# turlando/flac-py

Hardware: AMD Instinct MI355X
Metric: PCM samples/sec encode-analysis, 4608-blk/16-bit mono, 1/2/4/8 MI355X (higher is better)
Workload: dtype i16 in; f64 autocorrelation/Levinson; i32 predictors; 1 GPU; 1e6 synthetic mono 4608-sample int16 blocks, -l 12 -q 5 -r 0,5; units_per_gpu=1000000, units_total=1000000, block=4608, sample_bits=16, max_lpc_order=12, qlp_precision=5, mode=reference, parallelism=dp1 (block shards), open_eighths=0, lpc_pruning=on: candidates proven to lose skipped (sign bound, partial-sum tiers)

## Files before the change

flac-py_amd/csrc/flacmi_host.cpp:

```cpp
#include <dlfcn.h>
#include <hip/hip_runtime.h>

#include <algorithm>
#include <atomic>
#include <cerrno>
#include <chrono>
#include <cmath>
#include <cstdarg>
#include <cstdio>
#include <cstdlib>
#include <cstring>
#include <map>
#include <mutex>
#include <string>
#include <vector>

#include "../../include/flacmi.h"
#include "flacmi_kernels.h"
#include "pymath.h"
#include "device_common.h"

using namespace flacmi;

static double (*volatile libm_cos)(double) = cos;
// ... 414 lines not shown
static int use_mfma() {
    static const int v = [] {
        const char* e = getenv("FLACMI_NO_MFMA");
        return (e && atoi(e) != 0) ? 0 : 1;
    }();
    return v;
}

static int use_stream() {
    static const int v = [] {
        const char* e = getenv("FLACMI_NO_STREAM");
        return (e && atoi(e) != 0) ? 0 : 1;
    }();
    return v;
}

static int sign_bound_allowed() {
    static const int v = [] {
        const char* e = getenv("FLACMI_NO_SIGNBOUND");
        return (e && atoi(e) != 0) ? 0 : 1;
    }();
    return v;
}

static int prune_allowed() {
    static const int v = [] {
        const char* e = getenv("FLACMI_NO_PRUNE");
        return (e && atoi(e) != 0) ? 0 : 1;
    }();
    return v;
}

constexpr int64_t kOverlapMinUnits = 16384;
static int overlap_mode() { return knob(kKnobOverlap); }

static int analyze_device_impl(flacmi_ctx* ctx, const flacmi_batch* b, const flacmi_params* p,
                               const flacmi_outputs* o, hipStream_t s, bool allow_overlap = true) {
    if (int rc = set_device(ctx)) return rc;
    const bool lpc = p->mode == FLACMI_MODE_REFERENCE || p->mode == FLACMI_MODE_LPC_ONLY;
    const int L = lpc ? p->max_lpc_order : 0;
    const int rec_words = FLACMI_LPC_REC_WORDS(L);
    if (lpc) {
        if (int rc = ensure_buf(ctx->rec, sizeof(int32_t) * (size_t)rec_words * (size_t)(b->n_units > 0 ? b->n_units : 1)))
            return rc;
    }
    const int energy = debug_stop() >= 11 ? 0 : knob(kKnobEnergyBound);
    const bool prune_call = p->mode == FLACMI_MODE_REFERENCE && !o->lpc_sums &&
                            !(p->reserved[1] & (FLACMI_FLAG_ALL_CANDIDATES | FLACMI_FLAG_LPC_SIGN)) && prune_allowed();
    const bool ebound = energy != 0 && prune_call && L >= 1 && L <= 12 && b->sample_bytes == 2 && p->qlp_precision <= 16;
    if (ebound) {
        if (int rc = ensure_buf(ctx->bound, sizeof(uint32_t) * 2 * (size_t)(b->n_units > 0 ? b->n_units : 1))) return rc;
    }
    constexpr int64_t kSubWords = 64 * 16;
    if (int rc = ensure_buf(ctx->retry, sizeof(int64_t) * (size_t)(kSubWords + 2 * b->n_units + 68))) return rc;
    struct Cls {
        int64_t unit0, count;
        int n;
    } cls[2];
    int ncls = 0;
    const int64_t nfull = b->n_units - b->n_tail_units;
    if (b->n_tail_units == 0 || b->tail_len == b->block_len) {
        cls[ncls++] = {0, b->n_units, b->block_len};
    } else {
        if (nfull > 0) cls[ncls++] = {0, nfull, b->block_len};
        cls[ncls++] = {nfull, b->n_tail_units, b->tail_len};
    }
// ... 26 lines not shown
                overlap = true;
                continue;
            }
        }
        int64_t k = overlap && ov > 1 ? cls[c].count / kOverlapMinUnits : 1;
        const int left = flacmi_ctx::kMaxChunks - nch - (ncls - 1 - c);
        k = k < 1 ? 1 : k > want ? want : k;
        k = k > left ? left : k;
        for (int64_t i = 0; i < k; ++i) {
            const int64_t u0 = cls[c].count * i / k, u1 = cls[c].count * (i + 1) / k;
            ch[nch++] = {cls[c].unit0 + u0, u1 - u0, cls[c].n};
        }
    }
    auto lpc_args = [&](const Chunk& k, LpcArgs& a) -> int {
        a = LpcArgs{};
        a.samples = b->samples;
        a.stride = b->unit_stride;
        a.unit0 = k.unit0;
        a.count = k.count;
        a.sample_bytes = b->sample_bytes;
        a.n = k.n;
        a.L = L;
        a.q = p->qlp_precision;
        a.lpc_sign = (p->reserved[1] & FLACMI_FLAG_LPC_SIGN) != 0;
        if (int rc = get_window(ctx, k.n, (double**)&a.window, &a.fuse_lo, &a.fuse_hi)) return rc;
        a.bound = ebound ? (uint32_t*)ctx->bound.p + 2 * k.unit0 : nullptr;
        if (b->sample_bits > 26) a.fuse_lo = a.fuse_hi = 0;
        a.log2thr = ctx->d_log2thr;
        a.rec = (int32_t*)ctx->rec.p + k.unit0 * rec_words;
        a.rec_words = rec_words;
        a.acf = o->acf ? o->acf + k.unit0 * 33 : nullptr;
        return 0;
    };
    auto launch_resid_chunk = [&](const Chunk& k, hipStream_t st) -> hipError_t {
        ResidArgs a{};
        a.samples = b->samples;
        a.stride = b->unit_stride;
        a.unit0 = k.unit0;
        a.count = k.count;
        a.sample_bytes = b->sample_bytes;
        a.n = k.n;
        a.L = L;
        a.mode = p->mode;
        a.rmin = p->rice_min;
        a.rmax = p->rice_max;
        a.rec = lpc ? (const int32_t*)ctx->rec.p + k.unit0 * rec_words : nullptr;
        a.rice_order = p->mode == FLACMI_MODE_RICE_ONLY ? p->reserved[0] : 0;
        a.rec_words = rec_words;
        a.log2thr = ctx->d_log2thr;
        a.meta = o->meta + k.unit0;
        a.rice_params = o->rice_params + k.unit0 * o->params_stride;
        a.params_stride = o->params_stride;
        a.residual = (char*)o->residual + (size_t)k.unit0 * o->residual_stride * o->residual_bytes;
        a.residual_stride = o->residual_stride;
        a.fixed_sums = o->fixed_sums ? o->fixed_sums + k.unit0 * 5 : nullptr;
        a.lpc_sums = o->lpc_sums ? o->lpc_sums + k.unit0 * 32 : nullptr;
        a.stop_after = debug_stop();
        a.mfma = use_mfma();
        int64_t* const rb = (int64_t*)ctx->retry.p;
        a.retry_sub = (unsigned long long*)rb;
        a.retry_count = (unsigned long long*)(rb + kSubWords);
        a.retry_list = rb + kSubWords + 2;
        a.retry2_count = (unsigned long long*)(rb + kSubWords + 2 + b->n_units + 64);
        a.retry2_list = rb + kSubWords + 4 + b->n_units + 64;
        a.sample_bits = b->sample_bits;
        a.stream = use_stream();
        a.prune = prune_call;
        if (ebound) {
            double* w = nullptr;
            if (get_window(ctx, k.n, &w, nullptr, nullptr, &a.chunk_weight)) return hipErrorOutOfMemory;
            a.bound = (const uint32_t*)ctx->bound.p + 2 * k.unit0;
            a.energy = energy;
        }
        a.sign_bound = !(p->reserved[1] & FLACMI_FLAG_TIERS_ONLY) && sign_bound_allowed();
        const bool wide = needs_wide(k.n, b->sample_bits, L, p->qlp_precision, p->mode);
        int path = (wide || o->residual_bytes == 8) ? 2 : (b->sample_bytes == 2 && p->qlp_precision <= 16) ? 0 : 1;
        if (path == 2 && o->residual_bytes == 4 && split_ok(b->sample_bits, L, p->qlp_precision)) path = 3;
        return launch_resid(a, path, o->residual_bytes, st);
    };
    const int slot = ctx->ncalls % flacmi_ctx::kRing;
    hipEvent_t* ev = ctx->ev[slot];
    hipStream_t side = nullptr;
    if (overlap && !allow_overlap) overlap = false;
    if (overlap) {
        if (int rc = enc_streams(ctx)) return rc;
        side = enc_side(ctx);
        if (side == s) overlap = false;
    }
    ctx->nchunks[slot] = overlap ? nch : 0;
    HIP_TRY(hipEventRecord(ev[0], s));
    if (overlap) {
        HIP_TRY(hipStreamWaitEvent(side, ev[0], 0));
        for (int i = 0; i < nch; ++i) {
            LpcArgs a;
            if (int rc = lpc_args(ch[i], a)) return rc;
            HIP_TRY(launch_lpc(a, side));
            HIP_TRY(hipEventRecord(ctx->lpc_done[i], side));
        }
        HIP_TRY(hipEventRecord(ev[1], side));
        for (int i = 0; i < nch; ++i) {
            HIP_TRY(hipStreamWaitEvent(s, ctx->lpc_done[i], 0));
            HIP_TRY(hipEventRecord(ev[3 + 2 * i], s));
            HIP_TRY(launch_resid_chunk(ch[i], s));
            HIP_TRY(hipEventRecord(ev[4 + 2 * i], s));
        }
    } else {
        for (int i = 0; i < nch && lpc; ++i) {
            LpcArgs a;
            if (int rc = lpc_args(ch[i], a)) return rc;
            HIP_TRY(launch_lpc(a, s));
        }
        HIP_TRY(hipEventRecord(ev[1], s));
        for (int i = 0; i < nch; ++i) HIP_TRY(launch_resid_chunk(ch[i], s));
    }
    HIP_TRY(hipEventRecord(ev[2], s));
    ctx->ncalls++;
    if (o->lpc_records) {
        if (lpc) {
            HIP_TRY(launch_expand_records((const int32_t*)ctx->rec.p, rec_words, L, b->n_units, o->lpc_records, s));
        } else {
            HIP_TRY(hipMemsetAsync(o->lpc_records, 0, sizeof(int32_t) * FLACMI_LPC_REC_WORDS(32) * b->n_units, s));
        }
    }
    return 0;
}

extern "C" {

int flacmi_analyze_device(flacmi_ctx* ctx, const flacmi_batch* batch, const flacmi_params* params,
                          const flacmi_outputs* out, void* stream) {
    if (!ctx) return fail(FLACMI_E_INVALID, "null context");
    if (int rc = validate(batch, params, out)) return rc;
    if (batch->n_units == 0) return 0;
    return analyze_device_impl(ctx, batch, params, out, (hipStream_t)stream);
}

int flacmi_analyze_host(flacmi_ctx* ctx, const flacmi_batch* batch, const flacmi_params* params,
// ... 1659 lines not shown
```

flac-py_amd/csrc/flacmi_kernels.h:

```cpp
#pragma once
#include <hip/hip_runtime.h>
#include <stdint.h>

#include "../../include/flacmi.h"

namespace flacmi {

constexpr int kWindowPad = 80;

struct LpcArgs {
    const void* samples;
    int64_t stride;
    int64_t unit0, count;
    int32_t sample_bytes;
    int32_t n, L, q;
    const double* window;
    const double* log2thr;
    int32_t* rec;
    int32_t rec_words;
    int32_t lpc_sign;
    double* acf;
    int32_t fuse_lo, fuse_hi;
    uint32_t* bound;
};
// ... 6 lines not shown
    const void* samples;
    int64_t stride;
    int64_t unit0, count;
    int32_t sample_bytes;
    int32_t n, L, mode;
    int32_t rmin, rmax;
    int32_t rice_order;
    const int32_t* rec;
    int32_t rec_words;
    const double* log2thr;
    flacmi_unit_meta* meta;
    int32_t* rice_params;
    int64_t params_stride;
    void* residual;
    int64_t residual_stride;
    int64_t* fixed_sums;
    int64_t* lpc_sums;
    int32_t stop_after;
    int32_t mfma;
    unsigned long long* retry_count;
    int64_t* retry_list;
    unsigned long long* retry2_count;
    int64_t* retry2_list;
    unsigned long long* retry_sub;
    int64_t retry_sub_cap;
    int32_t sample_bits;
    int32_t stream;
    int32_t prune;
    int32_t persist;
    int32_t sign_bound;
    const uint32_t* bound;
    const uint16_t* chunk_weight;
    int32_t energy;
};
#define FLACMI_STATUS_RETRY 0x7e

struct StereoChoice {
    int32_t code;
    int32_t status;
    int64_t unit[2];
};

struct FrameArgs {
    const void* samples;
    int64_t stride;
    int32_t sample_bytes;
    int32_t block_len, tail_len;
    int64_t n_units, n_tail_units;
    int32_t channels, sample_size, q;
    int64_t first_frame, n_frames;
    const flacmi_unit_meta* meta;
    const int32_t* rice_params;
    int64_t params_stride;
    const void* residual;
    int32_t residual_bytes;
    int64_t residual_stride;
    int64_t* offsets;
    int32_t* status;
    uint8_t* out;
    int64_t capacity;
    const uint16_t* crc_slice;
    const uint16_t* crc_pow;
    int32_t pack_split;
    unsigned long long* slow_count;
    int64_t* slow_list;
    int32_t ablate;
// ... 95 lines not shown
    uint8_t* parts;
    int32_t part_stride;
    const uint16_t* crc_slice;
    int32_t wasted_spec;
};

struct PcmArgs {
    const flacmi_pcm_frame* frames;
    int64_t n_frames;
    int32_t channels, bytes_per_sample, raw;
    uint8_t* out;
    int64_t capacity;
    int32_t* status;
};

struct ResidLaunch {
    int threads;
    size_t lds_bytes;
};

ResidLaunch resid_launch_config(int n, int rmax_eff, int residual_bytes);
constexpr int kMaxFinestParts = 4096;

enum Knob { kKnobOverlap = 0, kKnobMf8Grid, kKnobStreamGeneric, kKnobDecodeGeneric, kKnobPackGeneric, kKnobDecodeLpc, kKnobEnergyBound, kKnobInfoGrid, kKnobCount };
int knob(Knob k);

hipError_t launch_lpc(const LpcArgs& a, hipStream_t s);
int64_t lpc_units_per_round(const LpcArgs& a);
hipError_t launch_poison_lds(hipStream_t s);
hipError_t launch_export(const int64_t* off, const int32_t* st, int64_t nf, int64_t* h_off, int32_t* h_st,
                         hipStream_t s);
hipError_t launch_lpc_from_acf(const LpcArgs& a, hipStream_t s);
hipError_t launch_resid(const ResidArgs& a, int path, int residual_bytes, hipStream_t s);
hipError_t launch_expand_records(const int32_t* rec, int32_t rec_words, int32_t L, int64_t count,
                                 int32_t* out, hipStream_t s);
hipError_t launch_synth(void* dst, int32_t sample_bytes, int32_t bits, int64_t stride,
                        int64_t first_unit, int64_t n_units, int32_t len, uint64_t seed,
                        const int32_t* sintab, int32_t open8, hipStream_t s);
hipError_t launch_stats(const flacmi_unit_meta* meta, int64_t n_units, int32_t block_len,
                        int32_t tail_len, int64_t n_tail_units, int64_t* stats, hipStream_t s);

hipError_t launch_stereo_rows(const void* lr, int32_t sample_bytes, int64_t lr_stride, int64_t n_frames,
                              int32_t block_len, int32_t tail_len, int32_t has_tail, void* mid, int64_t mid_stride,
                              int32_t* side, int64_t side_stride, hipStream_t s);
hipError_t launch_wasted_rows(const void* in, int32_t sample_bytes, int64_t in_stride, int64_t n_units,
                              int32_t block_len, int32_t tail_len, int64_t n_tail_units, int32_t sample_bits,
                              void* out, int64_t out_stride, int32_t* wasted, hipStream_t s);
hipError_t launch_stereo_choose(const FrameArgs& a, hipStream_t s);

hipError_t launch_frame_sizes(const FrameArgs& a, int64_t* bsum, hipStream_t s);
int64_t frame_scan_blocks(int64_t n_frames);
hipError_t launch_pack(const FrameArgs& a, hipStream_t s);
hipError_t launch_decode(DecodeArgs a, hipStream_t s);
hipError_t launch_index(const IndexArgs& a, hipStream_t s);
hipError_t launch_frame_info(const InfoArgs& a, int grid_cap, hipStream_t s);
int64_t index_scan_groups(int64_t n_tiles);
hipError_t launch_pcm(const PcmArgs& a, hipStream_t s);

hipError_t launch_selftest(int32_t which, const double* x, double* out, int32_t* status, int64_t n,
                           const double* log2thr, hipStream_t s);

}
```

flac-py_amd/csrc/k_stream.hip:

```cpp
#include <type_traits>

#include "device_common.h"

namespace flacmi {

namespace {

typedef _Float16 h8 __attribute__((ext_vector_type(8)));
typedef float f4 __attribute__((ext_vector_type(4)));
typedef _Float16 h2 __attribute__((ext_vector_type(2)));
typedef unsigned short us2 __attribute__((ext_vector_type(2)));

#ifndef FLACMI_STREAM_CPT
#define FLACMI_STREAM_CPT 5
#endif
constexpr int kSCPT = FLACMI_STREAM_CPT;
#ifndef FLACMI_RICE_DEDUP
#define FLACMI_RICE_DEDUP 1
#endif
#ifndef FLACMI_SAD16
#define FLACMI_SAD16 1
#endif
__host__ __device__ constexpr int stream_threads(int n) {
    const int nch = n / 8;
    const int nt = 64 * ((nch + 64 * kSCPT - 1) / (64 * kSCPT));
    return nt < 64 ? 64 : nt;
}
constexpr int kSHP = 16;
constexpr uint32_t kMagicBits = 0x4B400000u;
constexpr int kRiceOrders = 8;

struct SLds {
    int xs, pk, rec, red, red2, red0, pks, total;
};

__host__ __device__ inline SLds stream_lds(int n, int nw, int tap_words, int P, int RS) {
    auto up = [](int b) { return (b + 15) & ~15; };
    auto mx = [](int x, int y) { return x > y ? x : y; };
    SLds l;
    int o = 0;
    l.xs = o;   o = up(o + 2 * (kSHP + n));
    l.pk = l.rec = o; o = up(o + mx(2 * P * RS, 4 * mx(tap_words, 1)));
    l.red = l.red2 = o; o = up(o + mx(8 * nw * 16, 8 * (nw + 1) * kRiceOrders));
    l.red0 = o; o = up(o + 8 * nw);
    l.pks = o;  o = up(o + 4 * P);
    l.total = o;
    return l;
}

__host__ __device__ constexpr int tap_table_words(int NG) { return NG > 0 ? 40 * NG + 1 : 0; }
__device__ __forceinline__ uint32_t f16_of_int(int v) {
    return (uint32_t)__builtin_bit_cast(unsigned short, (_Float16)(float)v);
}

constexpr uint32_t f16_bits(int v) {
    if (v == 0) return 0;
    const uint32_t sgn = v < 0 ? 0x8000u : 0u;
    const int m = v < 0 ? -v : v;
    int e = 0;
    while ((m >> (e + 1)) != 0) ++e;
    return sgn | (uint32_t)((e + 15) << 10) | (uint32_t)((m << (10 - e)) & 0x3ff);
}
constexpr int fixed_tap(int p, int j) {
    if (j == 0) return -1;
    if (j < 0 || j > p) return 0;
    int c = 1;
    for (int t = 0; t < j; ++t) c = c * (p - t) / (t + 1);
    return (j & 1) ? c : -c;
}
struct FixB {
    uint32_t w[64 * 4];
};
constexpr FixB make_fixb() {
    FixB t{};
    for (int l = 0; l < 64; ++l) {
        const int col = l & 15, kb = l >> 4, p = (col >> 2) + 1, rho = col & 3, ia = 12 + rho - 4 * kb;
        const int idx[2] = {ia, ia - 2};
        for (int k = 0; k < 2; ++k) {
            const int i = idx[k];
            t.w[4 * l + k] = f16_bits(256 * fixed_tap(p, i)) | f16_bits(256 * fixed_tap(p, i - 1)) << 16;
            t.w[4 * l + 2 + k] = f16_bits(fixed_tap(p, i)) | f16_bits(fixed_tap(p, i - 1)) << 16;
        }
    }
    return t;
}
__constant__ const FixB kFixB = make_fixb();

__device__ __forceinline__ uint32_t sad32(uint32_t a, uint32_t b, uint32_t acc) { return (a > b ? a - b : b - a) + acc; }
template <int CTRL>
__device__ __forceinline__ uint64_t dpp_min_u64(uint64_t v) {
    const uint32_t lo = (uint32_t)__builtin_amdgcn_update_dpp(0, (int)(uint32_t)v, CTRL, 0xf, 0xf, false);
    const uint32_t hi = (uint32_t)__builtin_amdgcn_update_dpp(0, (int)(uint32_t)(v >> 32), CTRL, 0xf, 0xf, false);
    const uint64_t o = ((uint64_t)hi << 32) | lo;
    return o < v ? o : v;
}
__device__ __forceinline__ uint32_t opaque(uint32_t v) {
    asm volatile("" : "+v"(v));
    return v;
}
__device__ __forceinline__ uint32_t opaque_s(uint32_t v) {
    asm volatile("" : "+s"(v));
    return v;
}

__device__ __forceinline__ uint32_t h2sub(uint32_t t, float c) {
    const h2 v = __builtin_bit_cast(h2, t) - h2{(_Float16)c, (_Float16)c};
    return __builtin_bit_cast(uint32_t, v);
}

__device__ __forceinline__ uint4 a_raw(uint2 q) {
    return uint4{__builtin_amdgcn_perm(0x64646464u, q.x, 0x04030401u), __builtin_amdgcn_perm(0x64646464u, q.y, 0x04030401u),
                 __builtin_amdgcn_perm(0x64646464u, q.x, 0x04020400u), __builtin_amdgcn_perm(0x64646464u, q.y, 0x04020400u)};
}
__device__ __forceinline__ h8 a_sub(uint4 r) {
    const uint4 v{h2sub(r.x, 1152.0f), h2sub(r.y, 1152.0f), h2sub(r.z, 1024.0f), h2sub(r.w, 1024.0f)};
    return __builtin_bit_cast(h8, v);
}

__device__ __forceinline__ int rice_param_exact(uint64_t s, int len) {
// ... 103 lines not shown

}

template <int NG, bool R05, int NFIX, bool LIST, bool EB, typename Args>
__device__ __forceinline__ void stream_unit(const Args& a, const int64_t gid, unsigned char* smem) {
    static_assert(!EB || (NG > 0 && !LIST), "the energy bound's build is the batch kernel's, in reference mode");
    const int tid = LIST ? (int)opaque((uint32_t)threadIdx.x) : (int)threadIdx.x, NT = NFIX ? stream_threads(NFIX) : (int)blockDim.x, lane = tid & 63, nw = NT >> 6;
#if FLACMI_STREAM_STAMPS
    uint64_t stamp[8];
    const uint64_t rt0 = __builtin_amdgcn_s_memrealtime();
    stamp[0] = __builtin_amdgcn_s_memtime();
#define STAMP(k) (stamp[k] = __builtin_amdgcn_s_memtime())
#else
#define STAMP(k) ((void)0)
#endif
    const int wid = __builtin_amdgcn_readfirstlane(tid >> 6);
    const int n = NFIX ? NFIX : a.n, L = NG > 0 ? (NFIX ? 4 * NG : a.L) : 0;
    const int nch = n >> 3, nblk = n >> 6;
    const int rw = NG > 0 ? (NFIX ? 2 + L + (L * (L + 1)) / 2 : a.rec_words) : 0;
    int rmax_eff = -1;
    for (int o = a.rmin; o <= a.rmax; ++o)
        if (n % (1 << o) == 0) rmax_eff = o;
    const int Pmax = 1 << rmax_eff;
    constexpr int RS = kRiceOrders;
    const SLds lay = stream_lds(n, nw, tap_table_words(NG), Pmax, RS);
    uint16_t* xs = reinterpret_cast<uint16_t*>(smem + lay.xs) + kSHP;
    int32_t* recl = reinterpret_cast<int32_t*>(smem + lay.rec);
    uint32_t* red0 = reinterpret_cast<uint32_t*>(smem + lay.red0);
    unsigned long long* red2 = reinterpret_cast<unsigned long long*>(smem + lay.red2);
    uint32_t* pks = reinterpret_cast<uint32_t*>(smem + lay.pks);
    uint16_t* pkw = reinterpret_cast<uint16_t*>(smem + lay.pk);
    flacmi_unit_meta* meta = a.meta + gid;
    MetaVals mv{};

    constexpr int kTW = tap_table_words(NG), kTJ = NG > 0 ? (kTW + 63) / 64 : 0;
    uint4 fixb;
    {
        const uint4* src = reinterpret_cast<const uint4*>((const int16_t*)a.samples + (a.unit0 + gid) * a.stride);
        uint4 q[kSCPT];
#pragma unroll
        for (int j = 0; j < kSCPT; ++j) {
#if FLACMI_NT_LOAD
            typedef unsigned int v4u __attribute__((ext_vector_type(4)));
            const v4u t = __builtin_nontemporal_load(reinterpret_cast<const v4u*>(src) + min(tid + j * NT, nch - 1));
            q[j] = uint4{t.x, t.y, t.z, t.w};
#else
            q[j] = src[min(tid + j * NT, nch - 1)];
#endif
        }
        fixb = reinterpret_cast<const uint4*>(kFixB.w)[lane];
        uint32_t cwv[EB ? kSCPT : 1];
        if constexpr (EB) {
#pragma unroll
            for (int j = 0; j < kSCPT; ++j) cwv[j] = a.chunk_weight[min(tid + j * NT, nch - 1)];
        }
        int32_t tv[kTJ > 0 ? kTJ : 1][2];
        if constexpr (NG > 0 && !EB) {
            const int32_t* r = a.rec + gid * rw;
#pragma unroll
            for (int j = 0; j < kTJ; ++j) {
                if (j > 0 && j * NT >= kTW) break;
                const int gw = tid + j * NT, p = gw / 10 + 1, w = gw - 10 * (p - 1);
                const int pc = p < L ? p : L, base = 2 + L + (pc * (pc - 1)) / 2;
                tv[j][0] = r[w == 8 ? 1 + pc : min(max(base + 15 - 2 * w, 0), rw - 1)];
                tv[j][1] = r[min(max(base + 14 - 2 * w, 0), rw - 1)];
            }
        }
        if (tid < kSHP) xs[tid - kSHP] = 0x8000u;
        if (tid < Pmax) pks[tid] = a.stop_after == 10 ? (uint32_t)n * 40u : 0u;
#if FLACMI_SAD16
        const uint32_t k8000 = opaque(0x80008000u);
#else
        const uint32_t k8000 = opaque(0x8000u);
#endif
        uint32_t sumx = 0, wsum = 0;
#pragma unroll
        for (int j = 0; j < kSCPT; ++j) {
            const int v = tid + j * NT;
            if (v < nch) {
                const uint4 y{q[j].x ^ 0x80008000u, q[j].y ^ 0x80008000u, q[j].z ^ 0x80008000u, q[j].w ^ 0x80008000u};
                *reinterpret_cast<uint4*>(xs + 8 * v) = y;
                const uint32_t yd[4] = {y.x, y.y, y.z, y.w};
                if constexpr (EB) {
// ... 14 lines not shown
#endif
                    }
                }
            }
        }
        if constexpr (NG > 0 && !EB) {
            uint32_t* tt = reinterpret_cast<uint32_t*>(recl);
#pragma unroll
            for (int j = 0; j < kTJ; ++j) {
                if (j > 0 && j * NT >= kTW) break;
                const int gw = tid + j * NT, p = gw / 10 + 1, w = gw - 10 * (p - 1);
                if (gw < kTW) {
                    auto tap = [&](int i, int32_t c) -> uint32_t {
                        if (p > L || i < 0 || i > p) return 0u;
                        return f16_of_int(i == 0 ? -(1 << c) : c);
                    };
                    tt[gw] = tap(16 - 2 * w, tv[j][0]) | tap(15 - 2 * w, tv[j][1]) << 16;
                }
            }
        }
        const uint32_t sx = wave_sum_u32(sumx);
        if (lane == 0) red0[wid] = sx;
        if constexpr (EB) {
            const uint32_t sw = wave_sum_u32(wsum >> 3);
            if (lane == 0) red0[nw + wid] = sw;
        }
    }
    STAMP(1);
    __syncthreads();
    STAMP(2);
    uint32_t negmask = 0;
    const int32_t* __restrict__ grec = NG > 0 ? a.rec + gid * rw : nullptr;
    if constexpr (NG > 0) {
        const int st = grec[0];
        if (st != 0) {
            if (wid == 0) {
                mv.status = st & 0xffff;
                mv.site = st >> 16;
                store_meta(meta, lane, mv, 0);
            }
            return;
        }
        if constexpr (!EB) negmask = (uint32_t)grec[1];
    }
    uint2 bw{0u, 0u};
    if constexpr (EB) bw = *reinterpret_cast<const uint2*>(a.bound + 2 * gid);
    const bool listed = EB && bw.x == kBoundUnusable && bw.y == kBoundOutside;

    const bool prune = EB || (NG > 0 && a.prune && !LIST);
    unsigned long long* red64 = reinterpret_cast<unsigned long long*>(smem + lay.red);
    auto lane_total = [&](bool with_lpc = true) __attribute__((always_inline)) -> uint64_t {
        uint64_t t = 0;
        int g = -1, o4l = 0;
        if (lane >= 1 && lane <= 4) {
            g = 0;
            o4l = lane - 1;
        } else if (NG > 0 && with_lpc && lane >= 16 && lane < 16 + 4 * NG) {
            g = 1 + ((lane - 16) >> 2);
            o4l = (lane - 16) & 3;
        }
        if (g >= 0) {
#pragma unroll 1
            for (int w2 = 0; w2 < nw; ++w2) t += red64[(w2 * 4 + g) * 4 + o4l];
        } else if (lane == 0) {
#pragma unroll 1
            for (int w2 = 0; w2 < nw; ++w2) t += red0[w2];
        }
        return t;
    };
    uint64_t tj = 0;
    bool pruned = false;
    {
        const int col = lane & 15, kb = lane >> 4, o4 = col >> 2, rho = col & 3;
        h8 B[NG + 1];
        int shg[NG + 1];
        const uint32_t* tt = reinterpret_cast<const uint32_t*>(recl);
        const int k0 = 4 + 4 * kb - rho;
        const uint32_t alb = 16u * (uint32_t)(k0 & 1);
        bool outside = false;
// ... 92 lines not shown
                            (g == 0 || !EX) ? sad32(bits, mbv, 0u) : lpc_abs(bits, shg[g], kgv, xn[r], 0u);
                        acc[g] += i >= start_of(g) ? sv : 0u;
                    } else if (g == 0 || !EX) {
                        acc[g] = opaque(sad32(bits, mbv, acc[g]));
                    } else {
                        acc[g] = lpc_abs(bits, shg[g], kgv, xn[r], acc[g]);
                    }
                }
            }
        };
        auto block = [&](auto g0c, auto g1c, auto exc, uint2 q, bool masked, int blk) __attribute__((always_inline)) {
            uint32_t xn[4];
            ldx(blk, xn);
            blockA(g0c, g1c, exc, a_raw(q), masked, xn);
        };
        const uint32_t xnone[4] = {0u, 0u, 0u, 0u};
        auto reduce_store = [&](auto g0c, auto bdc, auto g1c) __attribute__((always_inline)) {
            constexpr int G0 = decltype(g0c)::value, G1 = decltype(g1c)::value;
            constexpr bool BD = decltype(bdc)::value != 0;
#pragma unroll
            for (int g = G0; g <= G1; ++g) {
                uint32_t v = (BD && g > 0) ? acc[g] >> shg[g] : acc[g];
                v += (uint32_t)__builtin_amdgcn_update_dpp(0, (int)v, 0xB1, 0xf, 0xf, false);
                v += (uint32_t)__builtin_amdgcn_update_dpp(0, (int)v, 0x4E, 0xf, 0xf, false);
                uint64_t w = v;
                w += (uint64_t)(uint32_t)__builtin_amdgcn_ds_swizzle((int)v, 0x401F);
                w += __shfl_xor((unsigned long long)w, 32);
                if (rho == 0 && kb == 0) red64[(wid * 4 + g) * 4 + o4] = w;
            }
        };
        using I0 = std::integral_constant<int, 0>;
        using I1 = std::integral_constant<int, 1>;
        using ING = std::integral_constant<int, NG>;
        const int kw = (nblk - wid + nw - 1) / nw;
        if (EB && prune) {
            if (!listed) {
                for (int k = wid == 0 ? 1 : 0; k < kw; ++k) blockA(I0{}, I0{}, I0{}, a_raw(ld(wid + k * nw)), false, xnone);
                if (wid == 0) block(I0{}, I0{}, I0{}, ld0(), true, 0);
                reduce_store(I0{}, I0{}, I0{});
            }
        } else if (prune) {
            const bool no_lpc = a.stop_after == 12;
            for (int k = wid == 0 ? 1 : 0; k < kw; ++k) {
                const uint4 A = a_raw(ld(wid + k * nw));
                blockA(I0{}, I0{}, I0{}, A, false, xnone);
                if ((k & 3) == 0 && !no_lpc) blockA(I1{}, ING{}, I0{}, A, false, xnone);
            }
            if (wid == 0) block(I0{}, ING{}, I0{}, ld0(), true, 0);
            reduce_store(I0{}, I1{}, ING{});
        } else {
            for (int blk = wid == 0 ? nw : wid; blk < nblk; blk += nw) block(I0{}, ING{}, I1{}, ld(blk), false, blk);
            if (wid == 0) block(I0{}, ING{}, I1{}, ld0(), true, 0);
            reduce_store(I0{}, I0{}, ING{});
            if constexpr (LIST) mv.tiers = 1 | (1 << 8);
        }
        if (!listed) {
            __syncthreads();
            STAMP(3);
            tj = lane_total(!(EB && prune));
        }
        if constexpr (NG > 0) {
            if (prune) {
                uint64_t fk = (lane <= 4) ? (tj << 4) | (uint64_t)lane : ~0ull;
                fk = dpp_min_u64<0xB1>(fk);
                fk = dpp_min_u64<0x4E>(fk);
                fk = dpp_min_u64<0x141>(fk);
                fk = dpp_min_u64<0x140>(fk);
                const uint64_t fmin = ((uint64_t)(uint32_t)__builtin_amdgcn_readlane((int)(uint32_t)(fk >> 32), 0) << 28) |
                                      ((uint32_t)__builtin_amdgcn_readlane((int)(uint32_t)fk, 0) >> 4);
                bool tiers = true;
                if constexpr (EB) {
                    uint64_t wr = 0;
// ... 25 lines not shown
                                if (j > 0 && j * NT >= kTW) break;
                                const int gw = tid + j * NT, p = gw / 10 + 1, w = gw - 10 * (p - 1);
                                if (gw < kTW) {
                                    auto tap = [&](int i, int32_t c) -> uint32_t {
                                        if (p > L || i < 0 || i > p) return 0u;
                                        return f16_of_int(i == 0 ? -(1 << c) : c);
                                    };
                                    tw[gw] = tap(16 - 2 * w, tv[j][0]) | tap(15 - 2 * w, tv[j][1]) << 16;
                                }
                            }
                        }
                        __syncthreads();
#pragma unroll
                        for (int g = 1; g <= NG; ++g) {
                            const int p = 4 * (g - 1) + o4 + 1, wb = 10 * (p - 1) + (k0 >> 1);
                            const uint32_t w0 = tt[wb], w1 = tt[wb + 1], w2 = tt[wb + 2];
                            const uint32_t l0 = __builtin_amdgcn_alignbit(w1, w0, alb), l2 = __builtin_amdgcn_alignbit(w2, w1, alb);
                            const h2 k256{(_Float16)256.0f, (_Float16)256.0f};
                            const uint32_t h0 = __builtin_bit_cast(uint32_t, __builtin_bit_cast(h2, l0) * k256);
                            const uint32_t hh = __builtin_bit_cast(uint32_t, __builtin_bit_cast(h2, l2) * k256);
                            B[g] = __builtin_bit_cast(h8, uint4{h0, hh, l0, l2});
                            const h2 one{(_Float16)1.0f, (_Float16)1.0f};
                            float sw = __builtin_amdgcn_fdot2(__builtin_bit_cast(h2, l0 & 0x7fff7fffu), one, 0.0f, false);
                            sw = __builtin_amdgcn_fdot2(__builtin_bit_cast(h2, l2 & 0x7fff7fffu), one, sw, false);
                            sw += __shfl_xor(sw, 16);
                            sw += __shfl_xor(sw, 32);
                            outside |= rho == 0 && p <= L && sw > (float)kCoefLimit;
                            const uint32_t t0 = tt[10 * (p - 1) + 8] & 0xffffu;
                            shg[g] = p <= L ? (int)((t0 >> 10) & 31u) - 15 : 0;
                        }
                        if (__ballot(outside) || listed) {
                            if (tid == 0) {
                                meta->status = FLACMI_STATUS_RETRY;
                                const int r = (int)(gid & 63);
                                const unsigned long long k = atomicAdd(a.retry_sub + 16 * r, 1ull);
                                a.retry_list[r * a.retry_sub_cap + (int64_t)k] = gid;
                            }
                            return;
                        }
                        if (a.energy == 2) {
                            tiers = false;
                        } else {
                            for (int k = wid == 0 ? 4 : 0; k < kw; k += 4) blockA(I1{}, ING{}, I0{}, a_raw(ld(wid + k * nw)), false, xnone);
                            if (wid == 0) block(I1{}, ING{}, I0{}, ld0(), true, 0);
                            reduce_store(I1{}, I1{}, ING{});
                            __syncthreads();
                            tj = lane_total();
                        }
                    }
                }
#pragma unroll 1
                for (int t = 1; tiers; ++t) {
                    const uint64_t lb = tj > (uint64_t)n ? tj - (uint64_t)n : 0ull;
                    const uint64_t open = __ballot(lane >= 16 && lane < 16 + L && lb <= fmin);
                    pruned = open == 0 || a.stop_after >= 11;
                    mv.tiers = t | (4 << 8);
                    if (pruned || t == 4) break;
                    const uint32_t gneed = (uint32_t)(open >> 16);
                    __syncthreads();
                    for (int k = t == 1 ? 2 : t == 2 ? 1 : 3; k < kw; k += 4) {
                        const h8 A = a_sub(a_raw(ld(wid + k * nw)));
#pragma unroll
                        for (int g = 1; g <= NG; ++g) {
                            if ((gneed >> (4 * (g - 1))) & 15u) {
                                const f4 D = __builtin_amdgcn_mfma_f32_16x16x32_f16(A, B[g], C, 0, 0, 0);
#pragma unroll
                                for (int r = 0; r < 4; ++r) acc[g] = opaque(sad32(__float_as_uint(D[r]), mbv, acc[g]));
                            }
                        }
// ... 481 lines not shown
    if constexpr (NG > 0)
        if (!list && a.prune && a.energy != 0 && a.bound && a.chunk_weight) kern = k_resid_stream<NG, R05, NFIX, true>;
    hipError_t e = hipFuncSetAttribute((const void*)kern, hipFuncAttributeMaxDynamicSharedMemorySize, (int)lds);
    if (e != hipSuccess) return e;
    hipLaunchKernelGGL(kern, dim3(list ? stream_list_grid(a.count) : (unsigned)a.count), dim3(nt), lds, s, a);
    return hipGetLastError();
}

template <int NG, bool R05>
static hipError_t launch_stream_R(const ResidArgs& a, bool list, hipStream_t s) {
    if constexpr (R05)
        if (a.n == 4608 && (NG == 0 || a.L == 4 * NG) && knob(kKnobStreamGeneric) == 0)
            return launch_stream_K<NG, true, 4608>(a, list, s);
    return launch_stream_K<NG, R05, 0>(a, list, s);
}

template <int NG>
static hipError_t launch_stream_T(const ResidArgs& a, bool list, hipStream_t s) {
    int rmax_eff = -1;
    for (int o = a.rmin; o <= a.rmax; ++o)
        if (a.n % (1 << o) == 0) rmax_eff = o;
    const int maxord = NG > 0 && a.L > 4 ? a.L : 4;
    if (a.rmin == 0 && rmax_eff == 5 && (a.n >> 5) > maxord) return launch_stream_R<NG, true>(a, list, s);
    return launch_stream_R<NG, false>(a, list, s);
}

static hipError_t launch_stream_G(const ResidArgs& a, bool list, hipStream_t s) {
    if (a.mode == FLACMI_MODE_FIXED_ONLY) return launch_stream_T<0>(a, list, s);
    if (a.L <= 4) return launch_stream_T<1>(a, list, s);
    if (a.L <= 8) return launch_stream_T<2>(a, list, s);
    return launch_stream_T<3>(a, list, s);
}

hipError_t launch_resid_stream(const ResidArgs& a_in, hipStream_t s) {
    ResidArgs a = a_in;
    a.retry_sub_cap = (a.count + 63) / 64;
    hipError_t e = hipMemsetAsync(a.retry_sub, 0, 64 * 16 * sizeof(unsigned long long), s);
    if (e != hipSuccess) return e;
    if ((e = launch_stream_G(a, false, s)) != hipSuccess) return e;
    if (a.mode == FLACMI_MODE_FIXED_ONLY) return hipSuccess;
    if ((e = hipMemsetAsync(a.retry2_count, 0, sizeof(unsigned long long), s)) != hipSuccess) return e;
    if ((e = launch_poison_lds(s)) != hipSuccess) return e;
    if ((e = launch_stream_G(a, true, s)) != hipSuccess) return e;
    if ((e = launch_poison_lds(s)) != hipSuccess) return e;
    ResidArgs b = a;
    b.retry_count = a.retry2_count;
    b.retry_list = a.retry2_list;
    return a.L <= 8 ? launch_resid_retry_l8(b, s) : launch_resid_retry_l12(b, s);
}

}
```

Before: 460.5 billion samples/s.

## Merge per-chunk retry lists into class-wide lists and add stride-8 fixed MFMA path

After: 471.3 billion samples/s (median of 6 runs). 2.3% higher.

```diff
diff --git a/flac-py_amd/csrc/flacmi_host.cpp b/flac-py_amd/csrc/flacmi_host.cpp
--- a/flac-py_amd/csrc/flacmi_host.cpp
+++ b/flac-py_amd/csrc/flacmi_host.cpp
@@ -470,6 +470,9 @@
 }
 
 constexpr int64_t kOverlapMinUnits = 16384;
+#ifndef FLACMI_CLASS_LISTS
+#define FLACMI_CLASS_LISTS 1
+#endif
 static int overlap_mode() { return knob(kKnobOverlap); }
 
 static int analyze_device_impl(flacmi_ctx* ctx, const flacmi_batch* b, const flacmi_params* p,
@@ -562,8 +565,8 @@
         a.acf = o->acf ? o->acf + k.unit0 * 33 : nullptr;
         return 0;
     };
-    auto launch_resid_chunk = [&](const Chunk& k, hipStream_t st) -> hipError_t {
-        ResidArgs a{};
+    auto resid_args = [&](const Chunk& k, ResidArgs& a, int& path) -> hipError_t {
+        a = ResidArgs{};
         a.samples = b->samples;
         a.stride = b->unit_stride;
         a.unit0 = k.unit0;
@@ -604,8 +607,14 @@
         }
         a.sign_bound = !(p->reserved[1] & FLACMI_FLAG_TIERS_ONLY) && sign_bound_allowed();
         const bool wide = needs_wide(k.n, b->sample_bits, L, p->qlp_precision, p->mode);
-        int path = (wide || o->residual_bytes == 8) ? 2 : (b->sample_bytes == 2 && p->qlp_precision <= 16) ? 0 : 1;
+        path = (wide || o->residual_bytes == 8) ? 2 : (b->sample_bytes == 2 && p->qlp_precision <= 16) ? 0 : 1;
         if (path == 2 && o->residual_bytes == 4 && split_ok(b->sample_bits, L, p->qlp_precision)) path = 3;
+        return hipSuccess;
+    };
+    auto launch_resid_chunk = [&](const Chunk& k, hipStream_t st) -> hipError_t {
+        ResidArgs a;
+        int path = 0;
+        if (hipError_t e = resid_args(k, a, path); e != hipSuccess) return e;
         return launch_resid(a, path, o->residual_bytes, st);
     };
     const int slot = ctx->ncalls % flacmi_ctx::kRing;
@@ -628,11 +637,30 @@
             HIP_TRY(hipEventRecord(ctx->lpc_done[i], side));
         }
         HIP_TRY(hipEventRecord(ev[1], side));
-        for (int i = 0; i < nch; ++i) {
-            HIP_TRY(hipStreamWaitEvent(s, ctx->lpc_done[i], 0));
-            HIP_TRY(hipEventRecord(ev[3 + 2 * i], s));
-            HIP_TRY(launch_resid_chunk(ch[i], s));
-            HIP_TRY(hipEventRecord(ev[4 + 2 * i], s));
+        for (int i = 0; i < nch;) {
+            int j = i + 1;
+            while (j < nch && ch[j].n == ch[i].n && ch[j].unit0 == ch[j - 1].unit0 + ch[j - 1].count) ++j;
+            ResidArgs ca;
+            int cpath = 0;
+            const Chunk whole{ch[i].unit0, ch[j - 1].unit0 + ch[j - 1].count - ch[i].unit0, ch[i].n};
+            HIP_TRY(resid_args(whole, ca, cpath));
+            const bool merged = FLACMI_CLASS_LISTS && j - i > 1 && stream_class_ok(ca, cpath, o->residual_bytes);
+            for (int c = i; c < j; ++c) {
+                HIP_TRY(hipStreamWaitEvent(s, ctx->lpc_done[c], 0));
+                HIP_TRY(hipEventRecord(ev[3 + 2 * c], s));
+                if (merged) {
+                    ResidArgs a;
+                    int path = 0;
+                    HIP_TRY(resid_args(ch[c], a, path));
+                    if (c == i) HIP_TRY(launch_stream_class_begin(ca, s));
+                    HIP_TRY(launch_stream_class_batch(a, ch[c].unit0 - whole.unit0, whole.count, s));
+                    if (c == j - 1) HIP_TRY(launch_stream_class_lists(ca, s));
+                } else {
+                    HIP_TRY(launch_resid_chunk(ch[c], s));
+                }
+                HIP_TRY(hipEventRecord(ev[4 + 2 * c], s));
+            }
+            i = j;
         }
     } else {
         for (int i = 0; i < nch && lpc; ++i) {
diff --git a/flac-py_amd/csrc/flacmi_kernels.h b/flac-py_amd/csrc/flacmi_kernels.h
--- a/flac-py_amd/csrc/flacmi_kernels.h
+++ b/flac-py_amd/csrc/flacmi_kernels.h
@@ -62,6 +62,7 @@
     const uint32_t* bound;
     const uint16_t* chunk_weight;
     int32_t energy;
+    int64_t list_off;
 };
 #define FLACMI_STATUS_RETRY 0x7e
 
@@ -223,6 +224,10 @@
                          hipStream_t s);
 hipError_t launch_lpc_from_acf(const LpcArgs& a, hipStream_t s);
 hipError_t launch_resid(const ResidArgs& a, int path, int residual_bytes, hipStream_t s);
+bool stream_class_ok(const ResidArgs& cls, int path, int residual_bytes);
+hipError_t launch_stream_class_begin(const ResidArgs& cls, hipStream_t s);
+hipError_t launch_stream_class_batch(const ResidArgs& chunk, int64_t list_off, int64_t class_count, hipStream_t s);
+hipError_t launch_stream_class_lists(const ResidArgs& cls, hipStream_t s);
 hipError_t launch_expand_records(const int32_t* rec, int32_t rec_words, int32_t L, int64_t count,
                                  int32_t* out, hipStream_t s);
 hipError_t launch_synth(void* dst, int32_t sample_bytes, int32_t bits, int64_t stride,
diff --git a/flac-py_amd/csrc/k_stream.hip b/flac-py_amd/csrc/k_stream.hip
--- a/flac-py_amd/csrc/k_stream.hip
+++ b/flac-py_amd/csrc/k_stream.hip
@@ -20,6 +20,12 @@
 #endif
 #ifndef FLACMI_SAD16
 #define FLACMI_SAD16 1
+#endif
+#ifndef FLACMI_FIXED_STRIDE8
+#define FLACMI_FIXED_STRIDE8 1
+#endif
+#ifndef FLACMI_ENTRY_LOADS
+#define FLACMI_ENTRY_LOADS 1
 #endif
 __host__ __device__ constexpr int stream_threads(int n) {
     const int nch = n / 8;
@@ -85,6 +91,22 @@
     return t;
 }
 __constant__ const FixB kFixB = make_fixb();
+constexpr FixB make_fixb8(int t) {
+    FixB b{};
+    for (int l = 0; l < 64; ++l) {
+        const int col = l & 15, kb = l >> 4, p = 2 * t + (col >> 3) + 1, rho = col & 7, ia = 8 + rho - 4 * kb;
+        const int idx[2] = {ia, ia - 2};
+        for (int k = 0; k < 2; ++k) {
+            const int i = idx[k];
+            b.w[4 * l + k] = f16_bits(256 * fixed_tap(p, i)) | f16_bits(256 * fixed_tap(p, i - 1)) << 16;
+            b.w[4 * l + 2 + k] = f16_bits(fixed_tap(p, i)) | f16_bits(fixed_tap(p, i - 1)) << 16;
+        }
+    }
+    return b;
+}
+__constant__ const FixB kFixB8a = make_fixb8(0);
+__constant__ const FixB kFixB8b = make_fixb8(1);
+__device__ __forceinline__ uint4 fixb_of(uint32_t lane) { return reinterpret_cast<const uint4*>(kFixB.w)[lane]; }
 
 __device__ __forceinline__ uint32_t sad32(uint32_t a, uint32_t b, uint32_t acc) { return (a > b ? a - b : b - a) + acc; }
 template <int CTRL>
@@ -254,9 +276,18 @@
     uint16_t* pkw = reinterpret_cast<uint16_t*>(smem + lay.pk);
     flacmi_unit_meta* meta = a.meta + gid;
     MetaVals mv{};
+    constexpr bool S8 = FLACMI_FIXED_STRIDE8 && EB;
+    constexpr bool EL = FLACMI_ENTRY_LOADS && EB;
+    int st_entry = 0;
+    uint2 bw_entry{0u, 0u};
+    if constexpr (EL) {
+        st_entry = (a.rec + gid * rw)[0];
+        bw_entry = *reinterpret_cast<const uint2*>(a.bound + 2 * gid);
+    }
 
     constexpr int kTW = tap_table_words(NG), kTJ = NG > 0 ? (kTW + 63) / 64 : 0;
-    uint4 fixb;
+    uint4 fixb{};
+    uint4 fixb8[2]{};
     {
         const uint4* src = reinterpret_cast<const uint4*>((const int16_t*)a.samples + (a.unit0 + gid) * a.stride);
         uint4 q[kSCPT];
@@ -270,7 +301,17 @@
             q[j] = src[min(tid + j * NT, nch - 1)];
 #endif
         }
-        fixb = reinterpret_cast<const uint4*>(kFixB.w)[lane];
+        if constexpr (S8) {
+            fixb8[0] = reinterpret_cast<const uint4*>(kFixB8a.w)[lane];
+            fixb8[1] = reinterpret_cast<const uint4*>(kFixB8b.w)[lane];
+        } else {
+            fixb = reinterpret_cast<const uint4*>(kFixB.w)[lane];
+        }
+        if constexpr (EL) {
+            st_entry = (int)opaque_s((uint32_t)st_entry);
+            bw_entry.x = opaque_s(bw_entry.x);
+            bw_entry.y = opaque_s(bw_entry.y);
+        }
         uint32_t cwv[EB ? kSCPT : 1];
         if constexpr (EB) {
 #pragma unroll
@@ -351,7 +392,7 @@
     uint32_t negmask = 0;
     const int32_t* __restrict__ grec = NG > 0 ? a.rec + gid * rw : nullptr;
     if constexpr (NG > 0) {
-        const int st = grec[0];
+        const int st = EL ? st_entry : grec[0];
         if (st != 0) {
             if (wid == 0) {
                 mv.status = st & 0xffff;
@@ -363,7 +404,7 @@
         if constexpr (!EB) negmask = (uint32_t)grec[1];
     }
     uint2 bw{0u, 0u};
-    if constexpr (EB) bw = *reinterpret_cast<const uint2*>(a.bound + 2 * gid);
+    if constexpr (EB) bw = EL ? bw_entry : *reinterpret_cast<const uint2*>(a.bound + 2 * gid);
     const bool listed = EB && bw.x == kBoundUnusable && bw.y == kBoundOutside;
 
     const bool prune = EB || (NG > 0 && a.prune && !LIST);
@@ -522,12 +563,78 @@
         using I0 = std::integral_constant<int, 0>;
         using I1 = std::integral_constant<int, 1>;
         using ING = std::integral_constant<int, NG>;
+        auto fixed8 = [&]() __attribute__((always_inline)) {
+            const int o8 = col >> 3, rho8 = col & 7, nstep = n >> 7;
+            const h8 B8[2] = {__builtin_bit_cast(h8, fixb8[0]), __builtin_bit_cast(h8, fixb8[1])};
+            uint32_t acc8[2] = {0u, 0u};
+            const int eoff8 = 8 * (lane & 15) - 8 + 4 * kb;
+            auto ld8 = [&](int st) __attribute__((always_inline)) {
+                return *reinterpret_cast<const uint2*>(xs + 128 * st + eoff8);
+            };
+            auto step8 = [&](const uint4 Ar, bool masked) __attribute__((always_inline)) {
+                f4 D[2];
+#pragma unroll
+                for (int t = 0; t < 2; ++t) D[t] = __builtin_amdgcn_mfma_f32_16x16x32_f16(__builtin_bit_cast(h8, Ar), B8[t], C, 0, 0, 0);
+#pragma unroll
+                for (int t = 0; t < 2; ++t) {
+#pragma unroll
+                    for (int r = 0; r < 4; ++r) {
+                        const uint32_t bits = __float_as_uint(D[t][r]);
+                        if (masked) {
+                            const int i = 8 * (4 * kb + r) + rho8;
+                            acc8[t] += i >= 2 * t + o8 + 1 ? sad32(bits, mbv, 0u) : 0u;
+                        } else {
+                            acc8[t] = opaque(sad32(bits, mbv, acc8[t]));
+                        }
+                    }
+                }
+            };
+            int st = wid == 0 ? nw : wid;
+            for (; st + nw < nstep; st += 2 * nw) {
+                const uint2 q0 = ld8(st), q1 = ld8(st + nw);
+                step8(a_raw(q0), false);
+                step8(a_raw(q1), false);
+            }
+            if (st < nstep) step8(a_raw(ld8(st)), false);
+            if (wid == 0 && nstep > 0) {
+                const uint32_t t = opaque((uint32_t)tid);
+                step8(a_raw(*reinterpret_cast<const uint2*>(xs + 8 * (int)(t & 15) - 8 + 4 * (int)((t >> 4) & 3))), true);
+            }
+#pragma unroll
+            for (int t = 0; t < 2; ++t) {
+                uint32_t v = acc8[t];
+                v += (uint32_t)__builtin_amdgcn_update_dpp(0, (int)v, 0xB1, 0xf, 0xf, false);
+                v += (uint32_t)__builtin_amdgcn_update_dpp(0, (int)v, 0x4E, 0xf, 0xf, false);
+                v += (uint32_t)__builtin_amdgcn_update_dpp(0, (int)v, 0x141, 0xf, 0xf, false);
+                uint64_t w = v;
+                w += (uint64_t)(uint32_t)__builtin_amdgcn_ds_swizzle((int)v, 0x401F);
+                w += __shfl_xor((unsigned long long)w, 32);
+                if (rho8 == 0 && kb == 0) red64[(wid * 4 + 0) * 4 + 2 * t + o8] = w;
+            }
+            if ((n & 64) && wid == nstep % nw) {
+                const uint32_t t = opaque((uint32_t)tid);
+                B[0] = __builtin_bit_cast(h8, fixb_of(t & 63));
+                const uint2 q = *reinterpret_cast<const uint2*>(xs + 64 * (nblk - 1) + 4 * (int)(t & 15) - 12 + 4 * (int)((t >> 4) & 3));
+                blockA(I0{}, I0{}, I0{}, a_raw(q), nblk == 1, xnone);
+                uint32_t v = acc[0];
+                v += (uint32_t)__builtin_amdgcn_update_dpp(0, (int)v, 0xB1, 0xf, 0xf, false);
+                v += (uint32_t)__builtin_amdgcn_update_dpp(0, (int)v, 0x4E, 0xf, 0xf, false);
+                uint64_t w = v;
+                w += (uint64_t)(uint32_t)__builtin_amdgcn_ds_swizzle((int)v, 0x401F);
+                w += __shfl_xor((unsigned long long)w, 32);
+                if (rho == 0 && kb == 0) red64[(wid * 4 + 0) * 4 + o4] += w;
+            }
+        };
         const int kw = (nblk - wid + nw - 1) / nw;
         if (EB && prune) {
             if (!listed) {
-                for (int k = wid == 0 ? 1 : 0; k < kw; ++k) blockA(I0{}, I0{}, I0{}, a_raw(ld(wid + k * nw)), false, xnone);
-                if (wid == 0) block(I0{}, I0{}, I0{}, ld0(), true, 0);
-                reduce_store(I0{}, I0{}, I0{});
+                if constexpr (S8) {
+                    fixed8();
+                } else {
+                    for (int k = wid == 0 ? 1 : 0; k < kw; ++k) blockA(I0{}, I0{}, I0{}, a_raw(ld(wid + k * nw)), false, xnone);
+                    if (wid == 0) block(I0{}, I0{}, I0{}, ld0(), true, 0);
+                    reduce_store(I0{}, I0{}, I0{});
+                }
             }
         } else if (prune) {
             const bool no_lpc = a.stop_after == 12;
@@ -619,9 +726,10 @@
                         if (__ballot(outside) || listed) {
                             if (tid == 0) {
                                 meta->status = FLACMI_STATUS_RETRY;
-                                const int r = (int)(gid & 63);
+                                const int64_t id = gid + a.list_off;
+                                const int r = (int)(id & 63);
                                 const unsigned long long k = atomicAdd(a.retry_sub + 16 * r, 1ull);
-                                a.retry_list[r * a.retry_sub_cap + (int64_t)k] = gid;
+                                a.retry_list[r * a.retry_sub_cap + (int64_t)k] = id;
                             }
                             return;
                         }
@@ -1169,14 +1277,8 @@
     return launch_stream_T<3>(a, list, s);
 }
 
-hipError_t launch_resid_stream(const ResidArgs& a_in, hipStream_t s) {
-    ResidArgs a = a_in;
-    a.retry_sub_cap = (a.count + 63) / 64;
-    hipError_t e = hipMemsetAsync(a.retry_sub, 0, 64 * 16 * sizeof(unsigned long long), s);
-    if (e != hipSuccess) return e;
-    if ((e = launch_stream_G(a, false, s)) != hipSuccess) return e;
-    if (a.mode == FLACMI_MODE_FIXED_ONLY) return hipSuccess;
-    if ((e = hipMemsetAsync(a.retry2_count, 0, sizeof(unsigned long long), s)) != hipSuccess) return e;
+static hipError_t launch_stream_lists(const ResidArgs& a, hipStream_t s) {
+    hipError_t e;
     if ((e = launch_poison_lds(s)) != hipSuccess) return e;
     if ((e = launch_stream_G(a, true, s)) != hipSuccess) return e;
     if ((e = launch_poison_lds(s)) != hipSuccess) return e;
@@ -1186,4 +1288,40 @@
     return a.L <= 8 ? launch_resid_retry_l8(b, s) : launch_resid_retry_l12(b, s);
 }
 
-}
+hipError_t launch_resid_stream(const ResidArgs& a_in, hipStream_t s) {
+    ResidArgs a = a_in;
+    a.list_off = 0;
+    a.retry_sub_cap = (a.count + 63) / 64;
+    hipError_t e = hipMemsetAsync(a.retry_sub, 0, 64 * 16 * sizeof(unsigned long long), s);
+    if (e != hipSuccess) return e;
+    if ((e = launch_stream_G(a, false, s)) != hipSuccess) return e;
+    if (a.mode == FLACMI_MODE_FIXED_ONLY) return hipSuccess;
+    if ((e = hipMemsetAsync(a.retry2_count, 0, sizeof(unsigned long long), s)) != hipSuccess) return e;
+    return launch_stream_lists(a, s);
+}
+
+bool stream_class_ok(const ResidArgs& cls, int path, int residual_bytes) {
+    return stream_shape_ok(cls, path, residual_bytes) && cls.mode == FLACMI_MODE_REFERENCE && cls.prune && cls.energy != 0 &&
+           cls.bound && cls.chunk_weight;
+}
+hipError_t launch_stream_class_begin(const ResidArgs& cls, hipStream_t s) {
+    hipError_t e = hipMemsetAsync(cls.retry_sub, 0, 64 * 16 * sizeof(unsigned long long), s);
+    if (e != hipSuccess) return e;
+    return hipMemsetAsync(cls.retry2_count, 0, sizeof(unsigned long long), s);
+}
+hipError_t launch_stream_class_batch(const ResidArgs& chunk, int64_t list_off, int64_t class_count, hipStream_t s) {
+    if (chunk.count <= 0) return hipSuccess;
+    ResidArgs a = chunk;
+    a.list_off = list_off;
+    a.retry_sub_cap = (class_count + 63) / 64;
+    if (hipError_t e = launch_poison_lds(s); e != hipSuccess) return e;
+    return launch_stream_G(a, false, s);
+}
+hipError_t launch_stream_class_lists(const ResidArgs& cls, hipStream_t s) {
+    ResidArgs a = cls;
+    a.list_off = 0;
+    a.retry_sub_cap = (cls.count + 63) / 64;
+    return launch_stream_lists(a, s);
+}
+
+}
```
